# neuronika/neuronika

Hardware: NVIDIA H100
Metric: forward+backward GFLOP/s (higher is better)
Workload: dtype bf16

## Files before the change

### neuronika_b200/csrc/nk_gemm_tc.cu

```cuda
#include "nk_internal.cuh"
#include "nk_ptx.cuh"

namespace {

constexpr int BLOCK_M = 128;
constexpr int BLOCK_K = 64;
constexpr int WGMMA_K = 16;
constexpr int kNumThreads = 384;
constexpr uint32_t kSmemLimit = 232448;
constexpr int kEpiCols = 64;
constexpr uint32_t kEpiStageBytes = 2 * 64 * kEpiCols * 4;

struct GemmParams {
  int64_t M, N, K;
  int64_t ldc;
  void* C;
  const void* bias;
  float alpha, beta;
  int bias_bf16;
  int bias_per_row;
  int relu;
  const void* mask;
  float* colsum;
  int num_m_blocks, num_n_blocks, num_k_blocks;
  uint32_t a_lbo, a_sbo, a_kstep;
  uint32_t b_lbo, b_sbo, b_kstep;
  int rs_world, m_rot;
  int64_t rs_rows;
  void* rs_dst[8];
  int batch, a_batched, b_batched, batch_reduce, splits;
  int64_t c_batch_stride;
  int tma_store;
  int bias_stage;
  int64_t bias_batch_stride;
};

__device__ __forceinline__ int tile_m_block(const GemmParams& p, int tile) {
  const int t = tile % p.num_m_blocks;
  if (p.rs_world == 0) return t;
  const int owner = (t + p.m_rot) % p.rs_world;
  return owner * (p.num_m_blocks / p.rs_world) + t / p.rs_world;
}

constexpr int kGroupM = 16;
__device__ __forceinline__ void tile_coords(const GemmParams& p, int tile, int& m_blk, int& n_blk) {
  if (p.rs_world) {
    m_blk = tile_m_block(p, tile);
    n_blk = tile / p.num_m_blocks;
    return;
  }
  const int group_size = kGroupM * p.num_n_blocks;
  const int group = tile / group_size, in_group = tile - group * group_size;
  const int first_m = group * kGroupM;
  const int gm = min(p.num_m_blocks - first_m, kGroupM);
  m_blk = first_m + in_group % gm;
  n_blk = in_group / gm;
}

template <int BLOCK_N>
struct Cfg {
  static constexpr uint32_t A_BYTES = BLOCK_M * BLOCK_K * 2;
  static constexpr uint32_t B_BYTES = BLOCK_N * BLOCK_K * 2;
  static constexpr uint32_t STAGE_BYTES = A_BYTES + B_BYTES;
  static constexpr int kStagesMax = (kSmemLimit - 3072 - kEpiStageBytes) / STAGE_BYTES;
  static constexpr int kStages = kStagesMax > 8 ? 8 : kStagesMax;
  static constexpr uint32_t SMEM_BYTES = kStages * STAGE_BYTES + 3072 + kEpiStageBytes;
  static_assert(2 * BLOCK_N * 2 <= 1024, "bias slots");
};

__device__ __forceinline__ void scale_and_bias(const GemmParams& p, const void* bias, int64_t row, int64_t col0,
                                               const uint32_t* r, bool full, float* v) {
#pragma unroll
  for (int j = 0; j < 32; ++j) v[j] = __fmul_rn(p.alpha, __uint_as_float(r[j]));
  if (bias && p.bias_per_row) {
    const float b = p.bias_bf16 ? __bfloat162float(static_cast<const __nv_bfloat16*>(bias)[row]) : static_cast<const float*>(bias)[row];
#pragma unroll
    for (int j = 0; j < 32; ++j) v[j] += b;
  } else if (bias) {
    if (full && (reinterpret_cast<uintptr_t>(bias) & 15) == 0) {
      if (p.bias_bf16) {
        const uint4* bp = reinterpret_cast<const uint4*>(static_cast<const __nv_bfloat16*>(bias) + col0);
#pragma unroll
        for (int q = 0; q < 4; ++q) {
          const uint4 w = __ldg(bp + q);
          const uint32_t ww[4] = {w.x, w.y, w.z, w.w};
#pragma unroll
          for (int i = 0; i < 4; ++i) {
            v[q * 8 + 2 * i] += __uint_as_float(ww[i] << 16);
            v[q * 8 + 2 * i + 1] += __uint_as_float(ww[i] & 0xffff0000u);
          }
        }
      } else {
        const float4* bp = reinterpret_cast<const float4*>(static_cast<const float*>(bias) + col0);
#pragma unroll
        for (int q = 0; q < 8; ++q) {
          const float4 w = __ldg(bp + q);
          v[q * 4] += w.x, v[q * 4 + 1] += w.y, v[q * 4 + 2] += w.z, v[q * 4 + 3] += w.w;
        }
      }
    } else {
#pragma unroll
      for (int j = 0; j < 32; ++j)
        if (col0 + j < p.N)
          v[j] += p.bias_bf16 ? __bfloat162float(static_cast<const __nv_bfloat16*>(bias)[col0 + j])
                              : static_cast<const float*>(bias)[col0 + j];
    }
  }
}

template <typename TC>
__device__ __forceinline__ void epilogue_colsum_chunk32(const GemmParams& p, int64_t row, int64_t col0, const uint32_t* r,
                                                        int lane, bool vec_ok) {
  float v[32];
  const bool live = row < p.M;
  const TC* mrow = (p.mask && live) ? static_cast<const TC*>(p.mask) + row * p.ldc + col0 : nullptr;
  const bool full = col0 + 32 <= p.N;
#pragma unroll
  for (int j = 0; j < 32; ++j) v[j] = (live && col0 + j < p.N) ? p.alpha * __uint_as_float(r[j]) : 0.f;
  if (mrow) {
    if (full && vec_ok) {
      constexpr int V = 16 / sizeof(TC);
#pragma unroll
      for (int q = 0; q < 32 / V; ++q) {
        NkVec<TC> mk;
        mk.load(mrow + q * V);
#pragma unroll
        for (int i = 0; i < V; ++i) v[q * V + i] = mk.get(i) > 0.f ? v[q * V + i] : 0.f;
      }
    } else {
#pragma unroll
      for (int j = 0; j < 32; ++j)
        if (col0 + j < p.N) v[j] = nk_to_f32<TC>(mrow[j]) > 0.f ? v[j] : 0.f;
    }
  }
#pragma unroll
  for (int j = 0; j < 32; ++j) v[j] = nk_to_f32<TC>(nk_from_f32<TC>(v[j]));
#pragma unroll
  for (int off = 16; off >= 1; off >>= 1) {
    const bool upper = (lane & off) != 0;
#pragma unroll
    for (int i = 0; i < off; ++i) {
      const float send = upper ? v[i] : v[i + off];
      const float keep = upper ? v[i + off] : v[i];
      v[i] = keep + __shfl_xor_sync(0xffffffffu, send, off);
    }
  }
  if (col0 + lane < p.N) atomicAdd(p.colsum + col0 + lane, v[0]);
}

template <bool BATCH_BIAS>
__device__ __forceinline__ const void* batch_bias(const GemmParams& p, int64_t c_off) {
  if (!BATCH_BIAS || !c_off) return p.bias;
  return static_cast<const char*>(p.bias) + (c_off / p.c_batch_stride) * p.bias_batch_stride * (p.bias_bf16 ? 2 : 4);
}

template <typename TC, bool BATCH_BIAS>
__device__ __forceinline__ void epilogue_store_chunk32(const GemmParams& p, int64_t row, int64_t col0, const uint32_t* r,
                                                       int ncols, bool vec_ok, int64_t c_off, bool atomic) {
  TC* crow = static_cast<TC*>(p.C) + c_off + row * p.ldc + col0;
  if (atomic) {
    if constexpr (sizeof(TC) == 4) {
#pragma unroll
      for (int j = 0; j < 32; ++j)
        if (j < ncols && col0 + j < p.N) atomicAdd(reinterpret_cast<float*>(crow) + j, p.alpha * __uint_as_float(r[j]));
    }
    return;
  }
  if (p.rs_world) {
    const int owner = int(row / p.rs_rows);
    crow = static_cast<TC*>(p.rs_dst[owner]) + (row - owner * p.rs_rows) * p.ldc + col0;
  }
  float v[32];
  const bool full = (col0 + 32 <= p.N) && ncols == 32;
  scale_and_bias(p, batch_bias<BATCH_BIAS>(p, c_off), row, col0, r, full, v);
  const TC* mrow = p.mask ? static_cast<const TC*>(p.mask) + row * p.ldc + col0 : nullptr;
  if (full && vec_ok) {
    constexpr int V = 16 / sizeof(TC);
    if (mrow) {
#pragma unroll
      for (int q = 0; q < 32 / V; ++q) {
        NkVec<TC> mk;
        mk.load(mrow + q * V);
#pragma unroll
        for (int i = 0; i < V; ++i) v[q * V + i] = mk.get(i) > 0.f ? v[q * V + i] : 0.f;
      }
    }
    if (p.beta != 0.f) {
#pragma unroll
      for (int q = 0; q < 32 / V; ++q) {
        NkVec<TC> c;
        c.load(crow + q * V);
#pragma unroll
        for (int i = 0; i < V; ++i) v[q * V + i] += p.beta * c.get(i);
      }
    }
    if (p.relu) {
#pragma unroll
      for (int j = 0; j < 32; ++j) v[j] = v[j] > 0.f ? v[j] : 0.f;
    }
#pragma unroll
    for (int q = 0; q < 32 / V; ++q) {
      NkVec<TC> o;
#pragma unroll
      for (int i = 0; i < V; ++i) o.set(i, v[q * V + i]);
      o.store(crow + q * V);
    }
  } else {
#pragma unroll
    for (int j = 0; j < 32; ++j) {
      if (j < ncols && col0 + j < p.N) {
        float x = v[j];
        if (mrow) x = nk_to_f32<TC>(mrow[j]) > 0.f ? x : 0.f;
        if (p.beta != 0.f) x += p.beta * nk_to_f32<TC>(crow[j]);
        if (p.relu) x = x > 0.f ? x : 0.f;
        crow[j] = nk_from_f32<TC>(x);
      }
    }
  }
}

__device__ __forceinline__ int epi_index(int row, int col) {
  return row * kEpiCols + ((((col >> 2) ^ (row & 7))) << 2) + (col & 3);
}

__device__ __forceinline__ float col_bias(const GemmParams& p, int64_t col) {
  if (col >= p.N) return 0.f;
  return p.bias_bf16 ? __bfloat162float(static_cast<const __nv_bfloat16*>(p.bias)[col]) : static_cast<const float*>(p.bias)[col];
}

template <bool kAddBias>
__device__ __forceinline__ float epi_value(const GemmParams& p, float acc, float bias) {
  float v = __fmul_rn(p.alpha, acc);
  if (kAddBias) v += bias;
  return p.relu ? (v > 0.f ? v : 0.f) : v;
}

enum { kBiasNone, kBiasStaged, kBiasLoaded };

template <int BLOCK_N, typename TC, int kBias>
__device__ __forceinline__ void tma_store_tile(const GemmParams& p, const CUtensorMap* tmap_c, const float (&acc)[BLOCK_N / 2],
                                               int lane, int row0, int64_t n0, uint32_t stg0, uint32_t bias_s,
                                               uint32_t& store_buf) {
  constexpr int kStoreCols = 128 / int(sizeof(TC));
  const int r = lane >> 2;
  const int q = lane & 3;
  const int sm_row = (lane & 7) + ((lane >> 3) & 1) * 8;
  const int sm_blk = lane >> 4;
#pragma unroll
  for (int ch = 0; ch < BLOCK_N / kStoreCols; ++ch) {
    const uint32_t buf = stg0 + store_buf * (64 * 128);
    if (lane == 0) ptx::tma_store_wait_read<1>();
    __syncwarp();
    const int64_t col0 = n0 + ch * kStoreCols;
    uint32_t packed[4];
#pragma unroll
    for (int jj = 0; jj < kStoreCols / 8; ++jj) {
      const int j = (ch * (kStoreCols / 8) + jj) * 4;
      float b0 = 0.f, b1 = 0.f;
      if constexpr (kBias == kBiasStaged) {
        const uint32_t w = ptx::ld_shared_b32(bias_s + uint32_t(ch * kStoreCols + jj * 8 + 2 * q) * 2);
        b0 = __uint_as_float(w << 16), b1 = __uint_as_float(w & 0xffff0000u);
      } else if constexpr (kBias == kBiasLoaded) {
        const int64_t col = col0 + jj * 8 + 2 * q;
        b0 = col_bias(p, col), b1 = col_bias(p, col + 1);
      }
      constexpr bool kAdd = kBias != kBiasNone;
      const float v0 = epi_value<kAdd>(p, acc[j], b0), v1 = epi_value<kAdd>(p, acc[j + 1], b1);
      const float v2 = epi_value<kAdd>(p, acc[j + 2], b0), v3 = epi_value<kAdd>(p, acc[j + 3], b1);
      if constexpr (sizeof(TC) == 2) {
        const __nv_bfloat162 lo = __floats2bfloat162_rn(v0, v1), hi = __floats2bfloat162_rn(v2, v3);
        packed[2 * (jj & 1)] = *reinterpret_cast<const uint32_t*>(&lo);
        packed[2 * (jj & 1) + 1] = *reinterpret_cast<const uint32_t*>(&hi);
        if (jj & 1) {
          const uint32_t off = sm_row * 128 + (((jj - 1 + sm_blk) ^ (sm_row & 7)) << 4);
          ptx::stmatrix_x4(buf + off, packed[0], packed[1], packed[2], packed[3]);
        }
      } else {
        const uint32_t off = r * 128 + (((2 * jj + (q >> 1)) ^ r) << 4) + (q & 1) * 8;
        ptx::st_shared_v2_f32(buf + off, v0, v1);
        ptx::st_shared_v2_f32(buf + off + 8 * 128, v2, v3);
      }
    }
    ptx::fence_proxy_async();
    __syncwarp();
    if (lane == 0) {
      if (row0 < p.M && col0 < p.N) ptx::tma_store_2d(tmap_c, buf, int(col0), row0);
      ptx::tma_store_commit();
    }
    store_buf ^= 1u;
  }
}

template <int BLOCK_N, bool A_MN, bool B_MN, typename TC, bool BATCH = false, bool BATCH_BIAS = false>
__global__ void __launch_bounds__(kNumThreads, 1)
gemm_tc_kernel(const __grid_constant__ CUtensorMap tmap_a, const __grid_constant__ CUtensorMap tmap_b,
               const __grid_constant__ CUtensorMap tmap_c, const GemmParams p) {
  using C_ = Cfg<BLOCK_N>;
  constexpr int kStages = C_::kStages;
  constexpr int kStoreCols = 128 / int(sizeof(TC));
  constexpr bool kTmaStore = !BATCH && BLOCK_N % kStoreCols == 0;
  static_assert(2 * 2 * 64 * 128 <= kEpiStageBytes, "staging buffers");
  extern __shared__ uint8_t smem_raw[];
  const uint32_t smem_base = (ptx::smem_u32(smem_raw) + 1023u) & ~1023u;
  const uint32_t smem_a0 = smem_base;
  const uint32_t smem_b0 = smem_base + kStages * C_::A_BYTES;
  const uint32_t bar_base = smem_base + kStages * C_::STAGE_BYTES;
  auto full_bar = [&](int s) { return bar_base + 8u * s; };
  auto empty_bar = [&](int s) { return bar_base + 8u * (kStages + s); };
  auto bias_empty_bar = [&](int s) { return bar_base + 8u * (2 * kStages + s); };
  const uint32_t epi_stage = bar_base + 1024;
  float* epi = reinterpret_cast<float*>(smem_raw + (epi_stage - ptx::smem_u32(smem_raw)));
  auto bias_slot = [&](int s) { return epi_stage + kEpiStageBytes + uint32_t(s) * (BLOCK_N * 2); };
  const bool stage_bias = kTmaStore && p.tma_store && p.bias_stage;

  const int wg = threadIdx.x >> 7;
  const int lane = threadIdx.x & 31;

  if (threadIdx.x == 0) {
    ptx::prefetch_tmap(&tmap_a);
    ptx::prefetch_tmap(&tmap_b);
    if (kTmaStore && p.tma_store) ptx::prefetch_tmap(&tmap_c);
    for (int s = 0; s < kStages; ++s) {
      ptx::mbar_init(full_bar(s), 1);
      ptx::mbar_init(empty_bar(s), 2);
    }
    for (int s = 0; s < 2; ++s) ptx::mbar_init(bias_empty_bar(s), 8);
    ptx::fence_barrier_init();
  }
  __syncthreads();

  const int tiles_mn = p.num_m_blocks * p.num_n_blocks;
  const int num_tiles = BATCH ? tiles_mn * (p.batch_reduce ? p.splits : p.batch) : tiles_mn;
  auto batch_range = [&](int outer, int& b0, int& b1) {
    if (!p.batch_reduce) {
      b0 = outer, b1 = outer + 1;
    } else {
      const int per = (p.batch + p.splits - 1) / p.splits;
      b0 = outer * per;
      b1 = min(p.batch, b0 + per);
    }
  };

  if (wg == 0) {
    ptx::setmaxnreg_dec<40>();
    if (threadIdx.x == 0) {
      int stage = 0;
      uint32_t phase = 0;
      for (int tile = blockIdx.x, local = 0; tile < num_tiles; tile += gridDim.x, ++local) {
        int m_blk, n_blk, b0 = 0, b1 = 1;
        tile_coords(p, BATCH ? tile % tiles_mn : tile, m_blk, n_blk);
        if (BATCH) batch_range(tile / tiles_mn, b0, b1);
        const int m0 = m_blk * BLOCK_M, n0 = n_blk * BLOCK_N;
        for (int bb = b0; bb < b1; ++bb)
        for (int kb = 0; kb < p.num_k_blocks; ++kb) {
          ptx::mbar_wait_spin(empty_bar(stage), phase ^ 1u);
          if (stage_bias && kb == 0) {
            const int s = local & 1;
            const uint32_t bytes = 2u * uint32_t(min(int64_t(BLOCK_N), p.N - n0));
            ptx::mbar_wait_spin(bias_empty_bar(s), ((local >> 1) & 1) ^ 1u);
            ptx::mbar_expect_tx(full_bar(stage), C_::STAGE_BYTES + bytes);
            ptx::bulk_load(bias_slot(s), static_cast<const __nv_bfloat16*>(p.bias) + n0, bytes, full_bar(stage));
          } else {
            ptx::mbar_expect_tx(full_bar(stage), C_::STAGE_BYTES);
          }
          const int k0 = kb * BLOCK_K;
          const uint32_t sa = smem_a0 + stage * C_::A_BYTES;
          const uint32_t sb = smem_b0 + stage * C_::B_BYTES;
          if (A_MN) {
#pragma unroll
            for (int c = 0; c < BLOCK_M / 64; ++c) {
              if (BATCH && p.a_batched)
                ptx::tma_load_3d(sa + c * (64 * BLOCK_K * 2), &tmap_a, full_bar(stage), m0 + c * 64, k0, bb);
              else
                ptx::tma_load_2d(sa + c * (64 * BLOCK_K * 2), &tmap_a, full_bar(stage), m0 + c * 64, k0);
            }
          } else {
            if (BATCH && p.a_batched)
              ptx::tma_load_3d(sa, &tmap_a, full_bar(stage), k0, m0, bb);
            else
              ptx::tma_load_2d(sa, &tmap_a, full_bar(stage), k0, m0);
          }
          if (B_MN) {
#pragma unroll
            for (int c = 0; c < BLOCK_N / 64; ++c) {
              if (BATCH && p.b_batched)
                ptx::tma_load_3d(sb + c * (64 * BLOCK_K * 2), &tmap_b, full_bar(stage), n0 + c * 64, k0, bb);
              else
                ptx::tma_load_2d(sb + c * (64 * BLOCK_K * 2), &tmap_b, full_bar(stage), n0 + c * 64, k0);
            }
          } else {
            if (BATCH && p.b_batched)
              ptx::tma_load_3d(sb, &tmap_b, full_bar(stage), k0, n0, bb);
            else
              ptx::tma_load_2d(sb, &tmap_b, full_bar(stage), k0, n0);
          }
          if (++stage == kStages) {
            stage = 0;
            phase ^= 1u;
          }
        }
      }
    }
    return;
  }

  ptx::setmaxnreg_inc<232>();
  const int cw = wg - 1;
  const int t = threadIdx.x & 127;
  const int warp = t >> 5;
  const bool vec_ok = ((p.ldc * int64_t(sizeof(TC))) % 16 == 0) && ((reinterpret_cast<uintptr_t>(p.C) & 15) == 0) &&
                      ((reinterpret_cast<uintptr_t>(p.mask) & 15) == 0);
  float* stg = epi + cw * (64 * kEpiCols);
  const uint32_t a_off = uint32_t(cw) * (64 * BLOCK_K * 2);
  float acc[BLOCK_N / 2];
  int stage = 0;
  uint32_t phase = 0;
  uint32_t store_buf = 0;
  for (int tile = blockIdx.x, local = 0; tile < num_tiles; tile += gridDim.x, ++local) {
    int m_blk, n_blk;
    tile_coords(p, BATCH ? tile % tiles_mn : tile, m_blk, n_blk);
    int k_total = p.num_k_blocks;
    if (BATCH) {
      int b0, b1;
      batch_range(tile / tiles_mn, b0, b1);
      k_total *= (b1 - b0);
    }
    int prev_stage = 0;
    for (int kb = 0; kb < k_total; ++kb) {
      ptx::mbar_wait_spin(full_bar(stage), phase);
      const uint64_t adesc = ptx::make_smem_desc_sw128(smem_a0 + stage * C_::A_BYTES + a_off, p.a_lbo, p.a_sbo);
      const uint64_t bdesc = ptx::make_smem_desc_sw128(smem_b0 + stage * C_::B_BYTES, p.b_lbo, p.b_sbo);
      ptx::fence_regs(acc);
      ptx::wgmma_fence();
#pragma unroll
      for (int k = 0; k < BLOCK_K / WGMMA_K; ++k)
        ptx::Wgmma<BLOCK_N>::template mma<int(A_MN), int(B_MN)>(acc, adesc + uint64_t((k * p.a_kstep) >> 4),
                                                                 bdesc + uint64_t((k * p.b_kstep) >> 4), (kb | k) != 0 ? 1u : 0u);
      ptx::wgmma_commit();
      ptx::wgmma_wait<1>();
      ptx::fence_regs(acc);
      if (kb > 0 && t == 0) ptx::mbar_arrive(empty_bar(prev_stage));
      prev_stage = stage;
      if (++stage == kStages) {
        stage = 0;
        phase ^= 1u;
      }
    }
    ptx::wgmma_wait<0>();
    ptx::fence_regs(acc);
    if (t == 0) ptx::mbar_arrive(empty_bar(prev_stage));

    if constexpr (kTmaStore) {
      if (p.tma_store) {
        const int row0 = m_blk * BLOCK_M + cw * 64 + warp * 16;
        const int64_t n0 = int64_t(n_blk) * BLOCK_N;
        const uint32_t stg0 = epi_stage + uint32_t(cw) * (2 * 64 * 128) + uint32_t(warp) * (16 * 128);
        const uint32_t bias_s = bias_slot(local & 1);
        if (stage_bias)
          tma_store_tile<BLOCK_N, TC, kBiasStaged>(p, &tmap_c, acc, lane, row0, n0, stg0, bias_s, store_buf);
        else if (p.bias)
          tma_store_tile<BLOCK_N, TC, kBiasLoaded>(p, &tmap_c, acc, lane, row0, n0, stg0, bias_s, store_buf);
        else
          tma_store_tile<BLOCK_N, TC, kBiasNone>(p, &tmap_c, acc, lane, row0, n0, stg0, bias_s, store_buf);
        if (stage_bias) {
          __syncwarp();
          if (lane == 0) ptx::mbar_arrive(bias_empty_bar(local & 1));
        }
        continue;
      }
    }

    const int64_t c_off = (BATCH && !p.batch_reduce) ? int64_t(tile / tiles_mn) * p.c_batch_stride : 0;
    const bool atomic = BATCH && p.batch_reduce;
    const int fr = warp * 16 + (lane >> 2);
    const int fc = (lane & 3) * 2;
    const int half = warp >> 1;
    const int rloc = (warp & 1) * 32 + lane;
    const int64_t row = int64_t(m_blk) * BLOCK_M + cw * 64 + rloc;
    constexpr int kChunks = (BLOCK_N + kEpiCols - 1) / kEpiCols;
#pragma unroll
    for (int ch = 0; ch < kChunks; ++ch) {
      constexpr int kFullBlocks = kEpiCols / 8;
      ptx::named_barrier(1 + cw, 128);
#pragma unroll
      for (int nb = 0; nb < kFullBlocks; ++nb) {
        if (ch * kFullBlocks + nb < BLOCK_N / 8) {
          const int j = (ch * kFullBlocks + nb) * 4;
          *reinterpret_cast<float2*>(stg + epi_index(fr, nb * 8 + fc)) = make_float2(acc[j], acc[j + 1]);
          *reinterpret_cast<float2*>(stg + epi_index(fr + 8, nb * 8 + fc)) = make_float2(acc[j + 2], acc[j + 3]);
        }
      }
      ptx::named_barrier(1 + cw, 128);
      const int chunk_cols = BLOCK_N - ch * kEpiCols < kEpiCols ? BLOCK_N - ch * kEpiCols : kEpiCols;
      if (!vec_ok && !p.colsum && !p.mask && !p.rs_world) {
        const int64_t col_base = int64_t(n_blk) * BLOCK_N + ch * kEpiCols;
        for (int rr = 0; rr < 16; ++rr) {
          const int srow = warp * 16 + rr;
          const int64_t grow = int64_t(m_blk) * BLOCK_M + cw * 64 + srow;
          if (grow >= p.M) break;
          const void* bias = p.bias;
          if constexpr (BATCH_BIAS) bias = batch_bias<true>(p, c_off);
          float rb = 0.f;
          if (bias && p.bias_per_row)
            rb = p.bias_bf16 ? __bfloat162float(static_cast<const __nv_bfloat16*>(bias)[grow]) : static_cast<const float*>(bias)[grow];
          for (int c = lane; c < chunk_cols; c += 32) {
            const int64_t col = col_base + c;
            if (col >= p.N) break;
            float v = __fmul_rn(p.alpha, stg[epi_index(srow, c)]);
            TC* cp = static_cast<TC*>(p.C) + c_off + grow * p.ldc + col;
            if (atomic) {
              if constexpr (sizeof(TC) == 4) atomicAdd(reinterpret_cast<float*>(cp), v);
              continue;
            }
            if (bias) {
              v += p.bias_per_row ? rb
                                  : (p.bias_bf16 ? __bfloat162float(static_cast<const __nv_bfloat16*>(bias)[col])
                                                 : static_cast<const float*>(bias)[col]);
            }
            if (p.beta != 0.f) v += p.beta * nk_to_f32<TC>(*cp);
            if (p.relu) v = v > 0.f ? v : 0.f;
            *cp = nk_from_f32<TC>(v);
          }
        }
        continue;
      }
      const int ncols = min(32, chunk_cols - half * 32);
      if (ncols > 0) {
        uint32_t r[32];
#pragma unroll
        for (int q = 0; q < 8; ++q) {
          float4 v = make_float4(0.f, 0.f, 0.f, 0.f);
          if (q * 4 < ncols) v = *reinterpret_cast<const float4*>(stg + epi_index(rloc, half * 32 + q * 4));
          r[4 * q] = __float_as_uint(v.x), r[4 * q + 1] = __float_as_uint(v.y);
          r[4 * q + 2] = __float_as_uint(v.z), r[4 * q + 3] = __float_as_uint(v.w);
        }
        const int64_t col0 = int64_t(n_blk) * BLOCK_N + ch * kEpiCols + half * 32;
        if (p.colsum && col0 < p.N) epilogue_colsum_chunk32<TC>(p, row, col0, r, lane, vec_ok);
        if (row < p.M && col0 < p.N) epilogue_store_chunk32<TC, BATCH_BIAS>(p, row, col0, r, ncols, vec_ok, c_off, atomic);
      }
    }
  }
  if (kTmaStore && p.tma_store && lane == 0) ptx::tma_store_wait<0>();
}

}

typedef CUresult (*EncodeTiledFn)(CUtensorMap*, CUtensorMapDataType, cuuint32_t, void*, const cuuint64_t*,
                                  const cuuint64_t*, const cuuint32_t*, const cuuint32_t*, CUtensorMapInterleave,
                                  CUtensorMapSwizzle, CUtensorMapL2promotion, CUtensorMapFloatOOBfill);

int make_tmap_2d(nk_ctx* ctx, CUtensorMap* tm, const void* base, int64_t rows, int64_t cols, int64_t ld,
                 uint32_t box_cols, uint32_t box_rows, int dtype) {
  if (!ctx->encode_tiled) return nk_set_error(ctx, NK_ERR_CUDA, "cuTensorMapEncodeTiled unavailable");
  cuuint64_t dims[2] = {(cuuint64_t)cols, (cuuint64_t)rows};
  cuuint64_t strides[1] = {(cuuint64_t)ld * nk_dtype_size(dtype)};
  cuuint32_t box[2] = {box_cols, box_rows};
  cuuint32_t estr[2] = {1, 1};
  CUresult r = reinterpret_cast<EncodeTiledFn>(ctx->encode_tiled)(
      tm, dtype == NK_BF16 ? CU_TENSOR_MAP_DATA_TYPE_BFLOAT16 : CU_TENSOR_MAP_DATA_TYPE_FLOAT32, 2,
      const_cast<void*>(base), dims, strides, box, estr,
      CU_TENSOR_MAP_INTERLEAVE_NONE, CU_TENSOR_MAP_SWIZZLE_128B, CU_TENSOR_MAP_L2_PROMOTION_L2_256B,
      CU_TENSOR_MAP_FLOAT_OOB_FILL_NONE);
  if (r != CUDA_SUCCESS)
    return nk_set_error(ctx, NK_ERR_CUDA, "cuTensorMapEncodeTiled failed (%d) rows=%lld cols=%lld ld=%lld", (int)r,
                        (long long)rows, (long long)cols, (long long)ld);
  return NK_OK;
}

namespace {

template <int BLOCK_N, bool A_MN, bool B_MN, typename TC, bool BATCH = false, bool BATCH_BIAS = false>
int launch_cfg(nk_ctx* ctx, const CUtensorMap& ta, const CUtensorMap& tb, const CUtensorMap& tc, GemmParams& p) {
  using C_ = Cfg<BLOCK_N>;
  auto kern = gemm_tc_kernel<BLOCK_N, A_MN, B_MN, TC, BATCH, BATCH_BIAS>;
  static bool attr_done[64] = {};
  if (!attr_done[ctx->device & 63]) {
    static_assert(C_::SMEM_BYTES <= kSmemLimit, "shared memory budget");
    NK_CUDA(ctx, cudaFuncSetAttribute(kern, cudaFuncAttributeMaxDynamicSharedMemorySize, (int)C_::SMEM_BYTES));
    attr_done[ctx->device & 63] = true;
  }
  p.num_n_blocks = int((p.N + BLOCK_N - 1) / BLOCK_N);
  int num_tiles = p.num_m_blocks * p.num_n_blocks;
  if (BATCH) {
    if (p.batch_reduce) {
      int want = (ctx->sm_count + num_tiles - 1) / num_tiles;
      if (want > p.batch) want = p.batch;
      const int per = (p.batch + want - 1) / want;
      p.splits = (p.batch + per - 1) / per;
      num_tiles *= p.splits;
    } else {
      num_tiles *= p.batch;
    }
  }
  const int units = ctx->sm_count;
  const int waves = (num_tiles + units - 1) / units;
  const int grid = (num_tiles + waves - 1) / waves;
  const size_t smem = C_::SMEM_BYTES;
  if (p.rs_world) {
    if (BLOCK_N != 256 || sizeof(TC) != 4 || p.N % 4 != 0)
      return nk_set_error(ctx, NK_ERR_UNSUPPORTED, "wgmma gemm: reduce-scatter epilogue needs 128x256 tiles, f32, N %% 4 == 0");
  }
  kern<<<grid, kNumThreads, smem, ctx->stream>>>(ta, tb, tc, p);
  ctx->launches++;
  cudaError_t le = cudaGetLastError();
  if (le != cudaSuccess)
    return nk_set_error(ctx, NK_ERR_CUDA, "launch of gemm_wgmma failed: %s (M=%lld N=%lld K=%lld BLOCK_N=%d grid=%d smem=%zu "
                        "a_mn=%d b_mn=%d out=%s)", cudaGetErrorString(le), (long long)p.M, (long long)p.N, (long long)p.K,
                        BLOCK_N, grid, smem, int(A_MN), int(B_MN), sizeof(TC) == 4 ? "f32" : "bf16");
  return NK_OK;
}

template <bool A_MN, bool B_MN, typename TC>
int launch_bn(nk_ctx* ctx, int block_n, const CUtensorMap& ta, const CUtensorMap& tb, const CUtensorMap& tc, GemmParams& p) {
  switch (block_n) {
    case 256: return launch_cfg<256, A_MN, B_MN, TC>(ctx, ta, tb, tc, p);
    case 128: return launch_cfg<128, A_MN, B_MN, TC>(ctx, ta, tb, tc, p);
    case 64: return launch_cfg<64, A_MN, B_MN, TC>(ctx, ta, tb, tc, p);
    default:
      if (!B_MN) {
        if (block_n == 32) return launch_cfg<32, A_MN, false, TC>(ctx, ta, tb, tc, p);
        if (block_n == 16) return launch_cfg<16, A_MN, false, TC>(ctx, ta, tb, tc, p);
      }
      return nk_set_error(ctx, NK_ERR_UNSUPPORTED, "wgmma gemm: unsupported BLOCK_N %d", block_n);
  }
}

}

bool nk_gemm_wgmma_supported(int transA, int transB, int64_t M, int64_t N, int64_t K, const void* A, int64_t lda,
                             const void* B, int64_t ldb) {
  (void)transA;
  (void)transB;
  if (M <= 0 || N <= 0 || K <= 0) return false;
  if ((reinterpret_cast<uintptr_t>(A) & 15) || (reinterpret_cast<uintptr_t>(B) & 15)) return false;
  if ((lda * 2) % 16 != 0 || (ldb * 2) % 16 != 0) return false;
  if (M > (int64_t(1) << 30) || N > (int64_t(1) << 30) || K > (int64_t(1) << 30)) return false;
  return true;
}

int nk_gemm_wgmma(nk_ctx* ctx, int transA, int transB, int64_t M, int64_t N, int64_t K, float alpha, const void* A,
                  int64_t lda, const void* B, int64_t ldb, float beta, void* C, int64_t ldc, int c_dtype,
                  const void* bias, int bias_dtype, int relu, const void* mask, float* colsum) {
  if (!nk_gemm_wgmma_supported(transA, transB, M, N, K, A, lda, B, ldb)) return NK_ERR_UNSUPPORTED;
  if (colsum && (N <= 16 || beta != 0.f)) return NK_ERR_UNSUPPORTED;
  const bool a_mn = transA != 0;
  const bool b_mn = transB == 0;
  int block_n = 256;
  if (N <= 16 && !b_mn)
    block_n = 16;
  else if (N <= 32 && !b_mn)
    block_n = 32;
  else if (N <= 64)
    block_n = 64;
  else if (N <= 128)
    block_n = 128;

  GemmParams p;
  p.M = M;
  p.N = N;
  p.K = K;
  p.ldc = ldc;
  p.C = C;
  p.bias = bias;
  p.alpha = alpha;
  p.beta = beta;
  p.bias_bf16 = bias_dtype == NK_BF16;
  p.bias_per_row = 0;
  p.relu = relu;
  p.mask = mask;
  p.colsum = colsum;
  p.batch = 1, p.a_batched = p.b_batched = p.batch_reduce = 0, p.splits = 1, p.c_batch_stride = 0, p.bias_batch_stride = 0;
  p.num_m_blocks = int((M + BLOCK_M - 1) / BLOCK_M);
  p.num_n_blocks = 0;
  p.num_k_blocks = int((K + BLOCK_K - 1) / BLOCK_K);
  p.rs_world = 0;
  p.m_rot = 0;
  p.rs_rows = M;
  for (int i = 0; i < 8; ++i) p.rs_dst[i] = nullptr;
  if (ctx->rs_world > 1) {
    if (M % (int64_t(ctx->rs_world) * BLOCK_M) != 0 || beta != 0.f || c_dtype != NK_F32)
      return nk_set_error(ctx, NK_ERR_INVALID_ARG, "wgmma gemm: reduce-scatter epilogue needs M %% (world*128) == 0, "
                          "beta == 0 and f32 output");
    p.rs_world = ctx->rs_world;
    p.rs_rows = M / ctx->rs_world;
    p.m_rot = ctx->rs_rank;
    for (int i = 0; i < ctx->rs_world; ++i) p.rs_dst[i] = ctx->rs_dst[i];
  }
  p.a_lbo = a_mn ? BLOCK_K * 128 : 16;
  p.a_sbo = 1024;
  p.a_kstep = a_mn ? WGMMA_K * 128 : WGMMA_K * 2;
  p.b_lbo = b_mn ? BLOCK_K * 128 : 16;
  p.b_sbo = 1024;
  p.b_kstep = b_mn ? WGMMA_K * 128 : WGMMA_K * 2;

  CUtensorMap ta, tb;
  int rc;
  if (a_mn)
    rc = make_tmap_2d(ctx, &ta, A, K, M, lda, 64, BLOCK_K);
  else
    rc = make_tmap_2d(ctx, &ta, A, M, K, lda, BLOCK_K, BLOCK_M);
  if (rc) return rc;
  if (b_mn)
    rc = make_tmap_2d(ctx, &tb, B, K, N, ldb, 64, BLOCK_K);
  else
    rc = make_tmap_2d(ctx, &tb, B, N, K, ldb, BLOCK_K, (uint32_t)block_n);
  if (rc) return rc;
  const int64_t c_size = int64_t(nk_dtype_size(c_dtype));
  CUtensorMap tc;
  memset(&tc, 0, sizeof(tc));
  p.tma_store = beta == 0.f && !mask && !colsum && !p.rs_world && (block_n * c_size) % 128 == 0 &&
                (reinterpret_cast<uintptr_t>(C) & 15) == 0 && (ldc * c_size) % 16 == 0 && (N * c_size) % 16 == 0;
  if (p.tma_store) {
    rc = make_tmap_2d(ctx, &tc, C, M, N, ldc, uint32_t(128 / c_size), 16, c_dtype);
    if (rc) return rc;
  }
  p.bias_stage = p.tma_store && bias && bias_dtype == NK_BF16 && (reinterpret_cast<uintptr_t>(bias) & 15) == 0 && N % 8 == 0;

  static const char* names[2][2][5] = {
      {{"wgmma_nt_128x256", "wgmma_nt_128x128", "wgmma_nt_128x64", "wgmma_nt_128x32", "wgmma_nt_128x16"},
       {"wgmma_nn_128x256", "wgmma_nn_128x128", "wgmma_nn_128x64", "", ""}},
      {{"wgmma_tt_128x256", "wgmma_tt_128x128", "wgmma_tt_128x64", "wgmma_tt_128x32", "wgmma_tt_128x16"},
       {"wgmma_tn_128x256", "wgmma_tn_128x128", "wgmma_tn_128x64", "", ""}}};
  const int bi = block_n == 256 ? 0 : block_n == 128 ? 1 : block_n == 64 ? 2 : block_n == 32 ? 3 : 4;
  ctx->last_gemm_kernel = names[a_mn][b_mn][bi];

#define NK_TC(AM, BM_)                                                              \
  (c_dtype == NK_BF16 ? launch_bn<AM, BM_, __nv_bfloat16>(ctx, block_n, ta, tb, tc, p) \
                      : launch_bn<AM, BM_, float>(ctx, block_n, ta, tb, tc, p))
  if (!a_mn && !b_mn) return NK_TC(false, false);
  if (!a_mn && b_mn) return NK_TC(false, true);
  if (a_mn && !b_mn) return NK_TC(true, false);
  return NK_TC(true, true);
#undef NK_TC
}

static int make_tmap_3d(nk_ctx* ctx, CUtensorMap* tm, const void* base, int64_t rows, int64_t cols, int64_t ld, int64_t batch,
                        int64_t batch_stride, uint32_t box_cols, uint32_t box_rows) {
  if (!ctx->encode_tiled) return nk_set_error(ctx, NK_ERR_CUDA, "cuTensorMapEncodeTiled unavailable");
  cuuint64_t dims[3] = {(cuuint64_t)cols, (cuuint64_t)rows, (cuuint64_t)batch};
  cuuint64_t strides[2] = {(cuuint64_t)ld * 2, (cuuint64_t)batch_stride * 2};
  cuuint32_t box[3] = {box_cols, box_rows, 1};
  cuuint32_t estr[3] = {1, 1, 1};
  CUresult r = reinterpret_cast<EncodeTiledFn>(ctx->encode_tiled)(
      tm, CU_TENSOR_MAP_DATA_TYPE_BFLOAT16, 3, const_cast<void*>(base), dims, strides, box, estr,
      CU_TENSOR_MAP_INTERLEAVE_NONE, CU_TENSOR_MAP_SWIZZLE_128B, CU_TENSOR_MAP_L2_PROMOTION_L2_256B,
      CU_TENSOR_MAP_FLOAT_OOB_FILL_NONE);
  if (r != CUDA_SUCCESS)
    return nk_set_error(ctx, NK_ERR_CUDA, "cuTensorMapEncodeTiled (3-d) failed (%d) rows=%lld cols=%lld ld=%lld batch=%lld stride=%lld",
                        (int)r, (long long)rows, (long long)cols, (long long)ld, (long long)batch, (long long)batch_stride);
  return NK_OK;
}

static int gemm_wgmma_batched(nk_ctx* ctx, int transA, int transB, int64_t M, int64_t N, int64_t K, float alpha, const void* A,
                              int64_t lda, int64_t strideA, const void* B, int64_t ldb, int64_t strideB, float beta, void* C,
                              int64_t ldc, int64_t strideC, int64_t batch, int c_dtype, const void* bias, int bias_dtype,
                              int bias_per_row, int64_t bias_stride, int relu, int reduce) {
  if (!nk_gemm_wgmma_supported(transA, transB, M, N, K, A, lda, B, ldb)) return NK_ERR_UNSUPPORTED;
  if (batch < 1 || batch > (int64_t(1) << 30) || (strideA * 2) % 16 != 0 || (strideB * 2) % 16 != 0) return NK_ERR_UNSUPPORTED;
  if (reduce && c_dtype != NK_F32) return NK_ERR_UNSUPPORTED;
  const bool a_mn = transA != 0, b_mn = transB == 0;
  int block_n = N <= 64 ? 64 : (N <= 128 ? 128 : 256);
  GemmParams p;
  p.M = M, p.N = N, p.K = K, p.ldc = ldc, p.C = C;
  p.bias = bias, p.bias_bf16 = bias_dtype == NK_BF16, p.bias_per_row = bias_per_row;
  p.bias_batch_stride = bias ? bias_stride : 0;
  p.alpha = alpha, p.beta = reduce ? 0.f : beta, p.relu = relu, p.mask = nullptr, p.colsum = nullptr;
  p.num_m_blocks = int((M + BLOCK_M - 1) / BLOCK_M);
  p.num_n_blocks = 0;
  p.num_k_blocks = int((K + BLOCK_K - 1) / BLOCK_K);
  p.rs_world = 0, p.m_rot = 0, p.rs_rows = M;
  for (int i = 0; i < 8; ++i) p.rs_dst[i] = nullptr;
  p.batch = int(batch), p.a_batched = strideA != 0, p.b_batched = strideB != 0, p.batch_reduce = reduce ? 1 : 0, p.splits = 1;
  p.c_batch_stride = strideC;
  p.tma_store = 0;
  p.bias_stage = 0;
  p.a_lbo = a_mn ? BLOCK_K * 128 : 16, p.a_sbo = 1024, p.a_kstep = a_mn ? WGMMA_K * 128 : WGMMA_K * 2;
  p.b_lbo = b_mn ? BLOCK_K * 128 : 16, p.b_sbo = 1024, p.b_kstep = b_mn ? WGMMA_K * 128 : WGMMA_K * 2;
  CUtensorMap ta, tb;
  int rc;
  if (p.a_batched)
    rc = a_mn ? make_tmap_3d(ctx, &ta, A, K, M, lda, batch, strideA, 64, BLOCK_K)
              : make_tmap_3d(ctx, &ta, A, M, K, lda, batch, strideA, BLOCK_K, BLOCK_M);
  else
    rc = a_mn ? make_tmap_2d(ctx, &ta, A, K, M, lda, 64, BLOCK_K) : make_tmap_2d(ctx, &ta, A, M, K, lda, BLOCK_K, BLOCK_M);
  if (rc) return rc;
  if (p.b_batched)
    rc = b_mn ? make_tmap_3d(ctx, &tb, B, K, N, ldb, batch, strideB, 64, BLOCK_K)
              : make_tmap_3d(ctx, &tb, B, N, K, ldb, batch, strideB, BLOCK_K, (uint32_t)block_n);
  else
    rc = b_mn ? make_tmap_2d(ctx, &tb, B, K, N, ldb, 64, BLOCK_K) : make_tmap_2d(ctx, &tb, B, N, K, ldb, BLOCK_K, (uint32_t)block_n);
  if (rc) return rc;
  CUtensorMap tc;
  memset(&tc, 0, sizeof(tc));
  ctx->last_gemm_kernel = "wgmma_batched";
  const bool per_batch_bias = p.bias && p.bias_batch_stride && !reduce;
#define NK_TCB(BN, AM, BM_)                                                                                      \
  (per_batch_bias ? (c_dtype == NK_BF16 ? launch_cfg<BN, AM, BM_, __nv_bfloat16, true, true>(ctx, ta, tb, tc, p) \
                                        : launch_cfg<BN, AM, BM_, float, true, true>(ctx, ta, tb, tc, p))        \
                  : (c_dtype == NK_BF16 ? launch_cfg<BN, AM, BM_, __nv_bfloat16, true>(ctx, ta, tb, tc, p)       \
                                        : launch_cfg<BN, AM, BM_, float, true>(ctx, ta, tb, tc, p)))
#define NK_TCB_BN(AM, BM_) (block_n == 256 ? NK_TCB(256, AM, BM_) : block_n == 128 ? NK_TCB(128, AM, BM_) : NK_TCB(64, AM, BM_))
  if (!a_mn && !b_mn) return NK_TCB_BN(false, false);
  if (!a_mn && b_mn) return NK_TCB_BN(false, true);
  if (a_mn && b_mn) return NK_TCB_BN(true, true);
  return nk_set_error(ctx, NK_ERR_UNSUPPORTED, "batched gemm: the TT form is not instantiated");
#undef NK_TCB_BN
#undef NK_TCB
}

int nk_gemm_wgmma_batched(nk_ctx* ctx, int transA, int transB, int64_t M, int64_t N, int64_t K, float alpha, const void* A,
                            int64_t lda, int64_t strideA, const void* B, int64_t ldb, int64_t strideB, void* C, int64_t ldc,
                            int64_t strideC, int64_t batch, int c_dtype, const void* row_bias, int bias_dtype, int relu,
                            int reduce) {
  return gemm_wgmma_batched(ctx, transA, transB, M, N, K, alpha, A, lda, strideA, B, ldb, strideB, 0.f, C, ldc, strideC, batch,
                            c_dtype, row_bias, bias_dtype, 1, 0, relu, reduce);
}

static bool f32_on_tensor_cores(const nk_ctx* ctx, int ab_dtype, int64_t K) {
  return ab_dtype == NK_F32 && ctx->f32_gemm != NK_F32_GEMM_IEEE && ctx->gemm_engine != NK_GEMM_SIMT && K > 0 &&
         ctx->rs_world == 0;
}

extern "C" {

int nk_gemm_bias_act(nk_ctx* ctx, int transA, int transB, int64_t M, int64_t N, int64_t K, float alpha,
                     const void* A, int64_t lda, const void* B, int64_t ldb, float beta, void* C, int64_t ldc,
                     int ab_dtype, int c_dtype, const void* bias, int bias_dtype, int relu) {
  if (!ctx) return NK_ERR_INVALID_ARG;
  NK_REQUIRE(ctx, nk_dtype_ok(ab_dtype) && nk_dtype_ok(c_dtype), "nk_gemm: bad dtype");
  NK_REQUIRE(ctx, M >= 0 && N >= 0 && K >= 0, "nk_gemm: negative dimension");
  if (M == 0 || N == 0) return NK_OK;
  NK_REQUIRE(ctx, C != nullptr && (K == 0 || (A && B)), "nk_gemm: NULL pointer");
  NK_REQUIRE(ctx, lda >= (transA ? M : K) && ldb >= (transB ? K : N) && ldc >= N,
             "nk_gemm: leading dimension too small (lda=%lld ldb=%lld ldc=%lld for M=%lld N=%lld K=%lld tA=%d tB=%d)",
             (long long)lda, (long long)ldb, (long long)ldc, (long long)M, (long long)N, (long long)K, transA, transB);
  NK_REQUIRE(ctx, !bias || nk_dtype_ok(bias_dtype), "nk_gemm: bad bias dtype");
  if (f32_on_tensor_cores(ctx, ab_dtype, K))
    return nk_gemm_tf32(ctx, transA, transB, M, N, K, alpha, A, lda, B, ldb, beta, C, ldc, c_dtype, bias, bias_dtype, relu);
  const bool want_tc = ab_dtype == NK_BF16 && ctx->gemm_engine != NK_GEMM_SIMT && K > 0;
  if (want_tc) {
    int rc = nk_gemm_wgmma(ctx, transA, transB, M, N, K, alpha, A, lda, B, ldb, beta, C, ldc, c_dtype, bias,
                             bias_dtype, relu, nullptr, nullptr);
    if (rc != NK_ERR_UNSUPPORTED) return rc;
    if (ctx->gemm_engine == NK_GEMM_TC)
      return nk_set_error(ctx, NK_ERR_UNSUPPORTED,
                          "nk_gemm: tensor-core engine forced but operands are not TMA-addressable "
                          "(16-byte aligned base, leading dimension multiple of 8 elements)");
  } else if (ctx->gemm_engine == NK_GEMM_TC) {
    return nk_set_error(ctx, NK_ERR_UNSUPPORTED, "nk_gemm: tensor-core engine forced but operands are not bf16");
  }
  return nk_gemm_simt(ctx, transA, transB, M, N, K, alpha, A, lda, B, ldb, beta, C, ldc, ab_dtype, c_dtype, bias,
                      bias_dtype, relu);
}

int nk_gemm_strided_batched(nk_ctx* ctx, int transA, int transB, int64_t M, int64_t N, int64_t K, float alpha, const void* A,
                            int64_t lda, int64_t strideA, const void* B, int64_t ldb, int64_t strideB, float beta, void* C,
                            int64_t ldc, int64_t strideC, int64_t batch, int ab_dtype, int c_dtype, const void* bias,
                            int64_t bias_stride, int bias_dtype) {
  if (!ctx) return NK_ERR_INVALID_ARG;
  NK_REQUIRE(ctx, nk_dtype_ok(ab_dtype) && nk_dtype_ok(c_dtype), "nk_gemm_strided_batched: bad dtype");
  NK_REQUIRE(ctx, M >= 0 && N >= 0 && K >= 0 && batch >= 0, "nk_gemm_strided_batched: negative dimension");
  NK_REQUIRE(ctx, !bias || nk_dtype_ok(bias_dtype), "nk_gemm_strided_batched: bad bias dtype");
  if (M == 0 || N == 0 || batch == 0) return NK_OK;
  const size_t cs = nk_dtype_size(c_dtype), bs = bias ? nk_dtype_size(bias_dtype) : 0;
  const bool tc = ab_dtype == NK_BF16 && ctx->gemm_engine != NK_GEMM_SIMT && K > 0 && !(transA && transB) &&
                  strideA >= 0 && strideB >= 0 && strideC >= 0 && bias_stride >= 0 && (strideC * int64_t(cs)) % 16 == 0 &&
                  (!bias || !bias_stride || batch == 1 || strideC > 0) &&
                  lda >= (transA ? M : K) && ldb >= (transB ? K : N) && ldc >= N;
  if (tc) {
    NK_REQUIRE(ctx, A && B && C, "nk_gemm_strided_batched: NULL pointer");
    const int rc = gemm_wgmma_batched(ctx, transA, transB, M, N, K, alpha, A, lda, strideA, B, ldb, strideB, beta, C, ldc,
                                      strideC, batch, c_dtype, bias, bias_dtype, 0, bias_stride, 0, 0);
    if (rc != NK_ERR_UNSUPPORTED) return rc;
  }
  const size_t as = nk_dtype_size(ab_dtype);
  for (int64_t b = 0; b < batch; ++b) {
    const int rc = nk_gemm_bias_act(
        ctx, transA, transB, M, N, K, alpha, A ? static_cast<const char*>(A) + b * strideA * int64_t(as) : nullptr, lda,
        B ? static_cast<const char*>(B) + b * strideB * int64_t(as) : nullptr, ldb, beta,
        C ? static_cast<char*>(C) + b * strideC * int64_t(cs) : nullptr, ldc, ab_dtype, c_dtype,
        bias ? static_cast<const char*>(bias) + b * bias_stride * int64_t(bs) : nullptr, bias_dtype, 0);
    if (rc) return rc;
// ... 57 lines not shown
```

Baseline: 771,200.

## Defer TMA-store of last epilogue chunks into next tile's mainloop

```diff
diff --git a/neuronika_b200/csrc/nk_gemm_tc.cu b/neuronika_b200/csrc/nk_gemm_tc.cu
--- a/neuronika_b200/csrc/nk_gemm_tc.cu
+++ b/neuronika_b200/csrc/nk_gemm_tc.cu
@@ -228,78 +228,123 @@
   return p.bias_bf16 ? __bfloat162float(static_cast<const __nv_bfloat16*>(p.bias)[col]) : static_cast<const float*>(p.bias)[col];
 }
 
-template <bool kAddBias>
+template <bool kAddBias, bool kScale, bool kRelu>
 __device__ __forceinline__ float epi_value(const GemmParams& p, float acc, float bias) {
-  float v = __fmul_rn(p.alpha, acc);
+  float v = kScale ? __fmul_rn(p.alpha, acc) : acc;
   if (kAddBias) v += bias;
-  return p.relu ? (v > 0.f ? v : 0.f) : v;
+  return kRelu ? (v > 0.f ? v : 0.f) : v;
 }
 
 enum { kBiasNone, kBiasStaged, kBiasLoaded };
 
-template <int BLOCK_N, typename TC, int kBias>
-__device__ __forceinline__ void tma_store_tile(const GemmParams& p, const CUtensorMap* tmap_c, const float (&acc)[BLOCK_N / 2],
-                                               int lane, int row0, int64_t n0, uint32_t stg0, uint32_t bias_s,
-                                               uint32_t& store_buf) {
+template <int BLOCK_N, typename TC, int kBias, bool kScale, bool kRelu>
+__device__ __forceinline__ void epi_chunk(const GemmParams& p, const float (&acc)[BLOCK_N / 2], int ch, int lane, int n0,
+                                          uint32_t bias_s, uint32_t (&w)[16]) {
   constexpr int kStoreCols = 128 / int(sizeof(TC));
-  const int r = lane >> 2;
   const int q = lane & 3;
-  const int sm_row = (lane & 7) + ((lane >> 3) & 1) * 8;
-  const int sm_blk = lane >> 4;
-#pragma unroll
-  for (int ch = 0; ch < BLOCK_N / kStoreCols; ++ch) {
-    const uint32_t buf = stg0 + store_buf * (64 * 128);
-    if (lane == 0) ptx::tma_store_wait_read<1>();
-    __syncwarp();
-    const int64_t col0 = n0 + ch * kStoreCols;
-    uint32_t packed[4];
-#pragma unroll
-    for (int jj = 0; jj < kStoreCols / 8; ++jj) {
-      const int j = (ch * (kStoreCols / 8) + jj) * 4;
-      float b0 = 0.f, b1 = 0.f;
-      if constexpr (kBias == kBiasStaged) {
-        const uint32_t w = ptx::ld_shared_b32(bias_s + uint32_t(ch * kStoreCols + jj * 8 + 2 * q) * 2);
-        b0 = __uint_as_float(w << 16), b1 = __uint_as_float(w & 0xffff0000u);
-      } else if constexpr (kBias == kBiasLoaded) {
-        const int64_t col = col0 + jj * 8 + 2 * q;
-        b0 = col_bias(p, col), b1 = col_bias(p, col + 1);
-      }
-      constexpr bool kAdd = kBias != kBiasNone;
-      const float v0 = epi_value<kAdd>(p, acc[j], b0), v1 = epi_value<kAdd>(p, acc[j + 1], b1);
-      const float v2 = epi_value<kAdd>(p, acc[j + 2], b0), v3 = epi_value<kAdd>(p, acc[j + 3], b1);
-      if constexpr (sizeof(TC) == 2) {
-        const __nv_bfloat162 lo = __floats2bfloat162_rn(v0, v1), hi = __floats2bfloat162_rn(v2, v3);
-        packed[2 * (jj & 1)] = *reinterpret_cast<const uint32_t*>(&lo);
-        packed[2 * (jj & 1) + 1] = *reinterpret_cast<const uint32_t*>(&hi);
-        if (jj & 1) {
-          const uint32_t off = sm_row * 128 + (((jj - 1 + sm_blk) ^ (sm_row & 7)) << 4);
-          ptx::stmatrix_x4(buf + off, packed[0], packed[1], packed[2], packed[3]);
-        }
-      } else {
-        const uint32_t off = r * 128 + (((2 * jj + (q >> 1)) ^ r) << 4) + (q & 1) * 8;
-        ptx::st_shared_v2_f32(buf + off, v0, v1);
-        ptx::st_shared_v2_f32(buf + off + 8 * 128, v2, v3);
-      }
-    }
-    ptx::fence_proxy_async();
-    __syncwarp();
-    if (lane == 0) {
-      if (row0 < p.M && col0 < p.N) ptx::tma_store_2d(tmap_c, buf, int(col0), row0);
-      ptx::tma_store_commit();
-    }
-    store_buf ^= 1u;
-  }
-}
-
-template <int BLOCK_N, bool A_MN, bool B_MN, typename TC, bool BATCH = false, bool BATCH_BIAS = false>
+#pragma unroll
+  for (int jj = 0; jj < kStoreCols / 8; ++jj) {
+    const int j = (ch * (kStoreCols / 8) + jj) * 4;
+    float b0 = 0.f, b1 = 0.f;
+    if constexpr (kBias == kBiasStaged) {
+      const uint32_t bw = ptx::ld_shared_b32(bias_s + uint32_t(ch * kStoreCols + jj * 8 + 2 * q) * 2);
+      b0 = __uint_as_float(bw << 16), b1 = __uint_as_float(bw & 0xffff0000u);
+    } else if constexpr (kBias == kBiasLoaded) {
+      const int64_t col = int64_t(n0) + ch * kStoreCols + jj * 8 + 2 * q;
+      b0 = col_bias(p, col), b1 = col_bias(p, col + 1);
+    }
+    constexpr bool kAdd = kBias != kBiasNone;
+    const float v0 = epi_value<kAdd, kScale, kRelu>(p, acc[j], b0), v1 = epi_value<kAdd, kScale, kRelu>(p, acc[j + 1], b1);
+    const float v2 = epi_value<kAdd, kScale, kRelu>(p, acc[j + 2], b0), v3 = epi_value<kAdd, kScale, kRelu>(p, acc[j + 3], b1);
+    if constexpr (sizeof(TC) == 2) {
+      const __nv_bfloat162 lo = __floats2bfloat162_rn(v0, v1), hi = __floats2bfloat162_rn(v2, v3);
+      w[2 * jj] = *reinterpret_cast<const uint32_t*>(&lo);
+      w[2 * jj + 1] = *reinterpret_cast<const uint32_t*>(&hi);
+    } else {
+      w[4 * jj] = __float_as_uint(v0), w[4 * jj + 1] = __float_as_uint(v1);
+      w[4 * jj + 2] = __float_as_uint(v2), w[4 * jj + 3] = __float_as_uint(v3);
+    }
+  }
+}
+
+template <typename TC>
+__device__ __forceinline__ void tma_store_chunk(const GemmParams& p, const CUtensorMap* tmap_c, const uint32_t (&w)[16],
+                                                int lane, int row0, int col0, uint32_t stg0, uint32_t& store_buf) {
+  const uint32_t buf = stg0 + store_buf * (64 * 128);
+  if (lane == 0) ptx::tma_store_wait_read<1>();
+  __syncwarp();
+  if constexpr (sizeof(TC) == 2) {
+    const int sm_row = (lane & 7) + ((lane >> 3) & 1) * 8;
+    const int sm_blk = lane >> 4;
+#pragma unroll
+    for (int jj = 0; jj < 8; jj += 2) {
+      const uint32_t off = sm_row * 128 + (((jj + sm_blk) ^ (sm_row & 7)) << 4);
+      ptx::stmatrix_x4(buf + off, w[2 * jj], w[2 * jj + 1], w[2 * jj + 2], w[2 * jj + 3]);
+    }
+  } else {
+    const int r = lane >> 2, q = lane & 3;
+#pragma unroll
+    for (int jj = 0; jj < 4; ++jj) {
+      const uint32_t off = r * 128 + (((2 * jj + (q >> 1)) ^ r) << 4) + (q & 1) * 8;
+      ptx::st_shared_v2_f32(buf + off, __uint_as_float(w[4 * jj]), __uint_as_float(w[4 * jj + 1]));
+      ptx::st_shared_v2_f32(buf + off + 8 * 128, __uint_as_float(w[4 * jj + 2]), __uint_as_float(w[4 * jj + 3]));
+    }
+  }
+  ptx::fence_proxy_async();
+  __syncwarp();
+  if (lane == 0) {
+    if (row0 < p.M && col0 < p.N) ptx::tma_store_2d(tmap_c, buf, col0, row0);
+    ptx::tma_store_commit();
+  }
+  store_buf ^= 1u;
+}
+
+template <int BLOCK_N, typename TC>
+struct CarryCfg {
+  static constexpr int kChunks = BLOCK_N / (128 / int(sizeof(TC)));
+  static constexpr int kCarry = sizeof(TC) == 2 ? kChunks : (kChunks + 1) / 2;
+  static constexpr int kFirst = kChunks - kCarry;
+};
+
+template <int BLOCK_N, typename TC, int kBias, bool kScale, bool kRelu>
+__device__ __forceinline__ void tma_store_convert(const GemmParams& p, const CUtensorMap* tmap_c,
+                                                  const float (&acc)[BLOCK_N / 2], int lane, int row0, int n0,
+                                                  uint32_t stg0, uint32_t bias_s, uint32_t& store_buf,
+                                                  uint32_t (&carry)[CarryCfg<BLOCK_N, TC>::kCarry][16]) {
+  using CC = CarryCfg<BLOCK_N, TC>;
+  constexpr int kStoreCols = 128 / int(sizeof(TC));
+#pragma unroll
+  for (int ch = 0; ch < CC::kFirst; ++ch) {
+    uint32_t w[16];
+    epi_chunk<BLOCK_N, TC, kBias, kScale, kRelu>(p, acc, ch, lane, n0, bias_s, w);
+    tma_store_chunk<TC>(p, tmap_c, w, lane, row0, n0 + ch * kStoreCols, stg0, store_buf);
+  }
+#pragma unroll
+  for (int c = 0; c < CC::kCarry; ++c)
+    epi_chunk<BLOCK_N, TC, kBias, kScale, kRelu>(p, acc, CC::kFirst + c, lane, n0, bias_s, carry[c]);
+}
+
+template <int BLOCK_N, typename TC, int kBias, typename... Args>
+__device__ __forceinline__ void tma_store_convert_any(const GemmParams& p, Args&&... args) {
+  if (p.alpha != 1.f) {
+    if (p.relu) tma_store_convert<BLOCK_N, TC, kBias, true, true>(p, args...);
+    else tma_store_convert<BLOCK_N, TC, kBias, true, false>(p, args...);
+  } else {
+    if (p.relu) tma_store_convert<BLOCK_N, TC, kBias, false, true>(p, args...);
+    else tma_store_convert<BLOCK_N, TC, kBias, false, false>(p, args...);
+  }
+}
+
+template <int BLOCK_N, bool A_MN, bool B_MN, typename TC, bool BATCH = false, bool BATCH_BIAS = false, bool TMA_STORE = false>
 __global__ void __launch_bounds__(kNumThreads, 1)
 gemm_tc_kernel(const __grid_constant__ CUtensorMap tmap_a, const __grid_constant__ CUtensorMap tmap_b,
                const __grid_constant__ CUtensorMap tmap_c, const GemmParams p) {
   using C_ = Cfg<BLOCK_N>;
   constexpr int kStages = C_::kStages;
   constexpr int kStoreCols = 128 / int(sizeof(TC));
-  constexpr bool kTmaStore = !BATCH && BLOCK_N % kStoreCols == 0;
+  static_assert(!TMA_STORE || (!BATCH && BLOCK_N % kStoreCols == 0), "TMA-store epilogue: whole chunks per tile");
   static_assert(2 * 2 * 64 * 128 <= kEpiStageBytes, "staging buffers");
+  using CC = CarryCfg<BLOCK_N, TC>;
   extern __shared__ uint8_t smem_raw[];
   const uint32_t smem_base = (ptx::smem_u32(smem_raw) + 1023u) & ~1023u;
   const uint32_t smem_a0 = smem_base;
@@ -311,7 +356,7 @@
   const uint32_t epi_stage = bar_base + 1024;
   float* epi = reinterpret_cast<float*>(smem_raw + (epi_stage - ptx::smem_u32(smem_raw)));
   auto bias_slot = [&](int s) { return epi_stage + kEpiStageBytes + uint32_t(s) * (BLOCK_N * 2); };
-  const bool stage_bias = kTmaStore && p.tma_store && p.bias_stage;
+  const bool stage_bias = TMA_STORE && p.bias_stage;
 
   const int wg = threadIdx.x >> 7;
   const int lane = threadIdx.x & 31;
@@ -319,7 +364,7 @@
   if (threadIdx.x == 0) {
     ptx::prefetch_tmap(&tmap_a);
     ptx::prefetch_tmap(&tmap_b);
-    if (kTmaStore && p.tma_store) ptx::prefetch_tmap(&tmap_c);
+    if (TMA_STORE) ptx::prefetch_tmap(&tmap_c);
     for (int s = 0; s < kStages; ++s) {
       ptx::mbar_init(full_bar(s), 1);
       ptx::mbar_init(empty_bar(s), 2);
@@ -416,7 +461,14 @@
   int stage = 0;
   uint32_t phase = 0;
   uint32_t store_buf = 0;
-  for (int tile = blockIdx.x, local = 0; tile < num_tiles; tile += gridDim.x, ++local) {
+  const uint32_t stg0 = epi_stage + uint32_t(cw) * (2 * 64 * 128) + uint32_t(warp) * (16 * 128);
+  uint32_t carry[TMA_STORE ? CC::kCarry : 1][16];
+  int carry_row0 = 0, carry_n0 = 0;
+  auto store_carried = [&](int c) {
+    tma_store_chunk<TC>(p, &tmap_c, carry[c], lane, carry_row0, carry_n0 + (CC::kFirst + c) * kStoreCols, stg0, store_buf);
+  };
+  int local = 0;
+  for (int tile = blockIdx.x; tile < num_tiles; tile += gridDim.x, ++local) {
     int m_blk, n_blk;
     tile_coords(p, BATCH ? tile % tiles_mn : tile, m_blk, n_blk);
     int k_total = p.num_k_blocks;
@@ -437,6 +489,11 @@
         ptx::Wgmma<BLOCK_N>::template mma<int(A_MN), int(B_MN)>(acc, adesc + uint64_t((k * p.a_kstep) >> 4),
                                                                  bdesc + uint64_t((k * p.b_kstep) >> 4), (kb | k) != 0 ? 1u : 0u);
       ptx::wgmma_commit();
+      if constexpr (TMA_STORE) {
+#pragma unroll
+        for (int c = 0; c < CC::kCarry; ++c)
+          if (local > 0 && kb == c) store_carried(c);
+      }
       ptx::wgmma_wait<1>();
       ptx::fence_regs(acc);
       if (kb > 0 && t == 0) ptx::mbar_arrive(empty_bar(prev_stage));
@@ -446,28 +503,31 @@
         phase ^= 1u;
       }
     }
+    if constexpr (TMA_STORE) {
+#pragma unroll
+      for (int c = 0; c < CC::kCarry; ++c)
+        if (local > 0 && c >= k_total) store_carried(c);
+    }
     ptx::wgmma_wait<0>();
     ptx::fence_regs(acc);
     if (t == 0) ptx::mbar_arrive(empty_bar(prev_stage));
 
-    if constexpr (kTmaStore) {
-      if (p.tma_store) {
-        const int row0 = m_blk * BLOCK_M + cw * 64 + warp * 16;
-        const int64_t n0 = int64_t(n_blk) * BLOCK_N;
-        const uint32_t stg0 = epi_stage + uint32_t(cw) * (2 * 64 * 128) + uint32_t(warp) * (16 * 128);
-        const uint32_t bias_s = bias_slot(local & 1);
-        if (stage_bias)
-          tma_store_tile<BLOCK_N, TC, kBiasStaged>(p, &tmap_c, acc, lane, row0, n0, stg0, bias_s, store_buf);
-        else if (p.bias)
-          tma_store_tile<BLOCK_N, TC, kBiasLoaded>(p, &tmap_c, acc, lane, row0, n0, stg0, bias_s, store_buf);
-        else
-          tma_store_tile<BLOCK_N, TC, kBiasNone>(p, &tmap_c, acc, lane, row0, n0, stg0, bias_s, store_buf);
-        if (stage_bias) {
-          __syncwarp();
-          if (lane == 0) ptx::mbar_arrive(bias_empty_bar(local & 1));
-        }
-        continue;
-      }
+    if constexpr (TMA_STORE) {
+      const int row0 = m_blk * BLOCK_M + cw * 64 + warp * 16;
+      const int n0 = n_blk * BLOCK_N;
+      const uint32_t bias_s = bias_slot(local & 1);
+      if (stage_bias)
+        tma_store_convert_any<BLOCK_N, TC, kBiasStaged>(p, &tmap_c, acc, lane, row0, n0, stg0, bias_s, store_buf, carry);
+      else if (p.bias)
+        tma_store_convert_any<BLOCK_N, TC, kBiasLoaded>(p, &tmap_c, acc, lane, row0, n0, stg0, bias_s, store_buf, carry);
+      else
+        tma_store_convert_any<BLOCK_N, TC, kBiasNone>(p, &tmap_c, acc, lane, row0, n0, stg0, bias_s, store_buf, carry);
+      if (stage_bias) {
+        __syncwarp();
+        if (lane == 0) ptx::mbar_arrive(bias_empty_bar(local & 1));
+      }
+      carry_row0 = row0, carry_n0 = n0;
+      continue;
     }
 
     const int64_t c_off = (BATCH && !p.batch_reduce) ? int64_t(tile / tiles_mn) * p.c_batch_stride : 0;
@@ -540,7 +600,13 @@
       }
     }
   }
-  if (kTmaStore && p.tma_store && lane == 0) ptx::tma_store_wait<0>();
+  if constexpr (TMA_STORE) {
+    if (local > 0) {
+#pragma unroll
+      for (int c = 0; c < CC::kCarry; ++c) store_carried(c);
+    }
+    if (lane == 0) ptx::tma_store_wait<0>();
+  }
 }
 
 }
@@ -572,12 +638,16 @@
 template <int BLOCK_N, bool A_MN, bool B_MN, typename TC, bool BATCH = false, bool BATCH_BIAS = false>
 int launch_cfg(nk_ctx* ctx, const CUtensorMap& ta, const CUtensorMap& tb, const CUtensorMap& tc, GemmParams& p) {
   using C_ = Cfg<BLOCK_N>;
-  auto kern = gemm_tc_kernel<BLOCK_N, A_MN, B_MN, TC, BATCH, BATCH_BIAS>;
-  static bool attr_done[64] = {};
-  if (!attr_done[ctx->device & 63]) {
+  constexpr bool kCanTmaStore = !BATCH && BLOCK_N % (128 / int(sizeof(TC))) == 0;
+  const bool tma_store = kCanTmaStore && p.tma_store;
+  auto kern = tma_store ? gemm_tc_kernel<BLOCK_N, A_MN, B_MN, TC, BATCH, BATCH_BIAS, kCanTmaStore>
+                        : gemm_tc_kernel<BLOCK_N, A_MN, B_MN, TC, BATCH, BATCH_BIAS>;
+  static bool attr_done[2][64] = {};
+  bool& attr = attr_done[tma_store][ctx->device & 63];
+  if (!attr) {
     static_assert(C_::SMEM_BYTES <= kSmemLimit, "shared memory budget");
     NK_CUDA(ctx, cudaFuncSetAttribute(kern, cudaFuncAttributeMaxDynamicSharedMemorySize, (int)C_::SMEM_BYTES));
-    attr_done[ctx->device & 63] = true;
+    attr = true;
   }
   p.num_n_blocks = int((p.N + BLOCK_N - 1) / BLOCK_N);
   int num_tiles = p.num_m_blocks * p.num_n_blocks;
```

New measurement: 784,500, median of 6. 1.7% higher.
